# JoshuaLim007/VoxelEngine

Hardware: AMD Instinct MI355X
Metric: Mrays/s primary+1-bounce @1080p, 8k×512×8k brickmap; % HBM roofline (higher is better)
Workload: dtype f32

## Files before the change

voxelengine_amd/csrc/vxrt_persist2.hpp:

```cpp
#pragma once

#include "vxrt_camera.hpp"
#include "vxrt_kernels.hpp"
#include "vxrt_pixel_map.hpp"
#include "vxrt_wave2.hpp"

namespace vxrt {

enum : uint32_t { PX_NONE = 0u, PX_PRIMARY = 1u, PX_SHADOW = 2u, PX_BOUNCE = 3u, PX_BOUNCE2 = 4u };

enum : int { PF_STAGE = 0, PF_TX, PF_ROW, PF_POS_X, PF_POS_Y, PF_POS_Z, PF_COL_X, PF_COL_Y, PF_COL_Z, PF_PCODE, PF_PSTEPS, PF_OCCL,
             PF_SAMPLE, PF_PIXEL_FIELDS };
enum : int { WV_COUNTERS = 0, WV_LIGHT_DX = 4, WV_LIGHT_DY, WV_LIGHT_DZ, WV_LIGHT_IVX, WV_LIGHT_IVY, WV_LIGHT_IVZ, WV_LIGHT_DN,
             WV_LIGHT_STEP_X, WV_LIGHT_STEP_Y, WV_LIGHT_STEP_Z, WV_SHADOW_FROM_END, WV_WORDS = 16 };
#ifndef VXRT_NO_KERNARG_RELOAD
#define VXRT_KERNARG_RELOAD 1
#endif
__device__ __forceinline__ const RenderArgs& kernarg_reload(const RenderArgs& in_registers)
{
#ifdef VXRT_KERNARG_RELOAD
    auto* p = (const __attribute__((address_space(4))) RenderArgs*)__builtin_amdgcn_kernarg_segment_ptr();
    asm volatile("" : "+s"(p));
    return *(const RenderArgs*)p;
#else
    return in_registers;
#endif
}

#ifndef VXRT_PERSIST2_OCC
#define VXRT_PERSIST2_OCC 5
#endif
#ifndef VXRT_QUEUE_GRANULE
#define VXRT_QUEUE_GRANULE 4u
#endif
#ifndef VXRT_SUBROUNDS2
#define VXRT_SUBROUNDS2 3
#endif
#ifndef VXRT_VOTE2_NEXT
#define VXRT_VOTE2_NEXT 2
#endif
#ifndef VXRT_VOTE2_END
#define VXRT_VOTE2_END 1
#endif
#ifndef VXRT_VOTE2_BOX
#define VXRT_VOTE2_BOX 2
#endif
#ifdef VXRT_VOTE2_ABS_BOX
__device__ __forceinline__ bool vote2(int parked, int others, int num, int k)
{
    (void)num;
    return parked >= k || (parked > 0 && others == 0);
}
#else
#define VXRT_VOTE2_ABS_BOX 0
#define VXRT_VOTE2_ABS_END 0
#define VXRT_VOTE2_ABS_NEXT 0
__device__ __forceinline__ bool vote2(int parked, int others, int num, int k)
{
    (void)k;
    return vote_run(parked, others, num);
}
#endif
#define PX_LD_U(f, v) do { if (LDS) v = PX[(f) * 64]; } while (0)
#define PX_ST_U(f, v) do { if (LDS) PX[(f) * 64] = (uint32_t)(v); } while (0)
#define PX_LD_I(f, v) do { if (LDS) v = (int)PX[(f) * 64]; } while (0)
#define PX_LD_F(f, v) do { if (LDS) v = __uint_as_float(PX[(f) * 64]); } while (0)
#define PX_ST_F(f, v) do { if (LDS) PX[(f) * 64] = __float_as_uint(v); } while (0)
#define PX_LD_POS() do { PX_LD_F(PF_POS_X, position.x); PX_LD_F(PF_POS_Y, position.y); PX_LD_F(PF_POS_Z, position.z); } while (0)
#define PX_ST_POS() do { PX_ST_F(PF_POS_X, position.x); PX_ST_F(PF_POS_Y, position.y); PX_ST_F(PF_POS_Z, position.z); } while (0)
#define PX_LD_COL() do { PX_LD_F(PF_COL_X, color.x); PX_LD_F(PF_COL_Y, color.y); PX_LD_F(PF_COL_Z, color.z); } while (0)
#define PX_ST_COL() do { PX_ST_F(PF_COL_X, color.x); PX_ST_F(PF_COL_Y, color.y); PX_ST_F(PF_COL_Z, color.z); } while (0)

template <bool STATS, bool BOUNCE2, bool MULTI, bool WIDE, bool COMMON = false>
__global__ __launch_bounds__(64, VXRT_PERSIST2_OCC) void k_render_persist2(RenderArgs A_kern)
{
    static_assert(!(COMMON && WIDE), "COMMON launches run on ordinary grids");
    using FT = FrameTraits<COMMON>;
    using Tracer = WaveTracerT<WIDE>;
    constexpr bool LDS = true;
    constexpr bool END_SHADOW = !(BOUNCE2 && MULTI) || COMMON;
    __shared__ uint32_t cold_block[(CF_TRACER_FIELDS + PF_PIXEL_FIELDS) * 64 + WV_WORDS];
    const WorldView& W = A_kern.W;
    const int lane = threadIdx.x & 63;
    uint32_t* const PX = &cold_block[CF_TRACER_FIELDS * 64 + lane];
    auto lane_view = [&](const RenderArgs& A, uint32_t v) -> LaneView {
        if (MULTI) {
            const ViewArgs& S = A.views[v];
            return LaneView{S.origin, S.fwd, S.up, S.right, S.frame_number, S.fb, S.color_aov, FT::hit_aov(S.hit_aov)};
        }
        return LaneView{A.origin, A.fwd, A.up, A.right, A.frame_number, A.fb, A.color_aov, FT::hit_aov(A.hit_aov)};
    };

    Tracer T;
    T.init(W, &cold_block[lane]);
    uint32_t stage = PX_NONE;
    uint32_t px_tx = 0, px_row = 0;
    f3 position = mk3(0, 0, 0), color = mk3(0, 0, 0);
    uint32_t pcode = 0;
    int p_steps = 0;
    float occl = 0.0f;
    int sample = 0;
    uint32_t n_primary = 0, n_shadow = 0, n_bounce = 0, n_hits = 0;
    PX_ST_U(PF_STAGE, stage);
    uint32_t* const WV = &cold_block[(CF_TRACER_FIELDS + PF_PIXEL_FIELDS) * 64];
    if (lane < 4)
        WV[WV_COUNTERS + lane] = 0u;
    {
        const f3 lu = A_kern.light_unit;
        const float dd = dot3(lu, lu);
        f3 ld = unit3_ordinary(lu, dd);
        const float ex = ld.x == 0 ? kFltEps : ld.x, ey = ld.y == 0 ? kFltEps : ld.y, ez = ld.z == 0 ? kFltEps : ld.z;
        float lix = rcp_rn(ex), liy = rcp_rn(ey), liz = rcp_rn(ez);
        if (!(ordinary(dd) & ordinary(ex) & ordinary(ey) & ordinary(ez))) {
            ld = unit3(lu);
            lix = 1.0f / (ld.x == 0 ? kFltEps : ld.x);
            liy = 1.0f / (ld.y == 0 ? kFltEps : ld.y);
            liz = 1.0f / (ld.z == 0 ? kFltEps : ld.z);
        }
        const bool light_special = !(fabsf(ld.x) >= kMinFastDir && fabsf(ld.y) >= kMinFastDir && fabsf(ld.z) >= kMinFastDir);
        const bool aov = FT::want_hit_aov(A_kern, MULTI);
        if (lane == 0) {
            WV[WV_LIGHT_DX] = __float_as_uint(ld.x);
            WV[WV_LIGHT_DY] = __float_as_uint(ld.y);
            WV[WV_LIGHT_DZ] = __float_as_uint(ld.z);
            WV[WV_LIGHT_IVX] = __float_as_uint(lix);
            WV[WV_LIGHT_IVY] = __float_as_uint(liy);
            WV[WV_LIGHT_IVZ] = __float_as_uint(liz);
            WV[WV_LIGHT_DN] = (ld.x > 0 ? 0u : 1u) | (ld.y > 0 ? 0u : 2u) | (ld.z > 0 ? 0u : 4u);
            WV[WV_LIGHT_STEP_X] = __float_as_uint(A_kern.light_step.x);
            WV[WV_LIGHT_STEP_Y] = __float_as_uint(A_kern.light_step.y);
            WV[WV_LIGHT_STEP_Z] = __float_as_uint(A_kern.light_step.z);
            WV[WV_SHADOW_FROM_END] = (END_SHADOW && FT::mode(A_kern) == 0 && A_kern.shadow && !light_special && !aov) ? 1u : 0u;
        }
    }

    uint32_t tile = 0, tile_used = 64u, tile_view = 0;
    uint32_t queue_shard = blockIdx.x % kQueueShards;
    bool drained = false;
    unsigned long long dg_iters = 0, dg_walk = 0, dg_drain = 0;
    unsigned int dg_runs[3] = {0, 0, 0}, dg_lanes[3] = {0, 0, 0};
    const unsigned long long dg_t0 = STATS ? wall_clock64() : 0ull;
    unsigned long long dg_next_ticks = 0, dg_park_ticks = 0;
    unsigned long long dg_co_runs = 0, dg_co_starts = 0;
    unsigned long long dg_end_shadow = 0;
#ifdef VXRT_TAIL_DEBUG
    unsigned long long px_t0 = 0;
#endif


    auto store_pixel = [&](const RenderArgs& A, const PixelCoords& pc, const LaneView& V, f3 origin, bool hit, f3 normal, f3 pos, f3 shaded) {
        PixelSink sink{A, pc.out_row, V.fb, V.color_aov};
        const int Wd = (int)A.width, Hd = (int)A.height;
        if (hit) {
            if (FT::mode(A) == 1) {
                f3 dv = pos - origin;
                float dist = sqrtf(dot3(dv, dv));
                const float wrap = (float)(1.0 + 1e-6);
                f3 hp = mk3(fmodf(pos.x / 128.0f, wrap), fmodf(pos.y / 128.0f, wrap), fmodf(pos.z / 128.0f, wrap));
                if (pc.x < (Wd >> 1) && pc.y < (Hd >> 1))
                    sink.put(pc.x, pc.y, normal);
                else if (pc.x >= (Wd >> 1) && pc.y < (Hd >> 1))
                    sink.put(pc.x, pc.y, hp);
                else if (pc.x < (Wd >> 1)) {
// ... 10 lines not shown
                    c = mk3(shaded.x / (shaded.x + 1.0f), shaded.y / (shaded.y + 1.0f), shaded.z / (shaded.z + 1.0f));
                c = mk3(lo(hi(c.x, 0), 1), lo(hi(c.y, 0), 1), lo(hi(c.z, 0), 1));
                sink.put(pc.x, pc.y, c);
            }
        } else {
            sink.put(pc.x, pc.y, shaded);
        }
        if (pc.tx == (A.width >> 1) && pc.ty == (A.height >> 1)) {
            float ten = 10.0f;
            pin(ten);
            sink.put(pc.x, pc.y, mk3(ten, ten, ten));
        }
        if (FT::mode(A) == 1 && pc.x < (Wd >> 1) && pc.y > (Hd >> 1))
            sink.put(pc.x, pc.y, mk3((float)p_steps / 256.0f, 0, 0));
    };

    auto shadow_from_end = [&](Tracer& Tr, const lanemask_t ended) -> lanemask_t {
        if (ended == 0ull)
            return 0ull;
        bool go = false;
        if (lane_test(ended)) {
            if (PX[PF_STAGE * 64] == PX_PRIMARY && WV[WV_SHADOW_FROM_END] != 0u) {
                TraceResult r;
                Tr.result(W, r);
                const f3 at = r.pos;
                const f3 from = at + mk3(__uint_as_float(WV[WV_LIGHT_STEP_X]), __uint_as_float(WV[WV_LIGHT_STEP_Y]),
                                         __uint_as_float(WV[WV_LIGHT_STEP_Z]));
                const f3 s0 = mk3(from.x * W.inv_f, from.y * W.inv_f, from.z * W.inv_f);
                const uint32_t signs = __float_as_uint(s0.x) | __float_as_uint(s0.y) | __float_as_uint(s0.z);
                if ((int32_t)signs >= 0 && s0.x < (float)W.cx && s0.y < (float)W.cy && s0.z < (float)W.cz) {
                    PX[PF_PCODE * 64] = r.ncode;
                    PX[PF_PSTEPS * 64] = (uint32_t)r.steps;
                    PX[PF_POS_X * 64] = __float_as_uint(at.x);
                    PX[PF_POS_Y * 64] = __float_as_uint(at.y);
                    PX[PF_POS_Z * 64] = __float_as_uint(at.z);
                    PX[PF_COL_X * 64] = 0u;
                    PX[PF_COL_Y * 64] = 0u;
                    PX[PF_COL_Z * 64] = 0u;
                    PX[PF_STAGE * 64] = PX_SHADOW;
                    Tr.cold[CF_RAY_CODES * 64] = (uint32_t)kMaxSteps << 7;
                    Tr.cold[CF_START_X * 64] = __float_as_uint(s0.x);
                    Tr.cold[CF_START_Y * 64] = __float_as_uint(s0.y);
                    Tr.cold[CF_START_Z * 64] = __float_as_uint(s0.z);
                    Tr.cold[CF_LAST_CI * 64] = 0xFFFFFFFFu;
                    Tr.cold[CF_TOTAL * 64] = 0u;
                    Tr.d = mk3(__uint_as_float(WV[WV_LIGHT_DX]), __uint_as_float(WV[WV_LIGHT_DY]), __uint_as_float(WV[WV_LIGHT_DZ]));
                    Tr.ivx = __uint_as_float(WV[WV_LIGHT_IVX]);
                    Tr.ivy = __uint_as_float(WV[WV_LIGHT_IVY]);
                    Tr.ivz = __uint_as_float(WV[WV_LIGHT_IVZ]);
                    Tr.dn = WV[WV_LIGHT_DN];
                    Tr.special = false;
                    Tr.st = ST_WALK;
                    go = true;
                }
            }
        }
        const lanemask_t launched = __ballot(go);
        const uint32_t n = (uint32_t)__popcll(launched);
        if (lane == 0) {
            WV[WV_COUNTERS + 1] += n;
            WV[WV_COUNTERS + 3] += n;
        }
        if (STATS)
            dg_end_shadow += n;
        return launched;
    };

    for (;;) {
        const unsigned long long m_walk = __ballot(T.st == ST_WALK);
        const unsigned long long m_box = __ballot(T.st == ST_BOX);
        const unsigned long long m_end = __ballot(waits_for_end(T.st));
        const unsigned long long m_next = __ballot(T.st == ST_DONE);
        if ((m_walk | m_box | m_end | m_next) == 0ull)
            break;
        const int n_walk = __popcll(m_walk), n_box = __popcll(m_box), n_end = __popcll(m_end), n_next = __popcll(m_next);
        if (STATS) {
            dg_iters += 1;
            dg_walk += (unsigned long long)n_walk;
            dg_drain += drained ? 1ull : 0ull;
        }

        int c_walk = n_walk, c_box = n_box, c_end = n_end, c_next = n_next;
        bool dg_end_ran = false, dg_end_restarted = false;
        if (vote2(c_box, c_walk, VXRT_VOTE2_BOX, VXRT_VOTE2_ABS_BOX)) {
            if (STATS) {
                dg_runs[2] += 1u;
                dg_lanes[2] += (unsigned)c_box;
                dg_park_ticks -= wall_clock64();
            }
            T.template phase_box<STATS>(W);
            if (STATS)
                dg_park_ticks += wall_clock64();
            c_box = 0;
            c_walk = __popcll(__ballot(T.st == ST_WALK));
            c_end = __popcll(__ballot(waits_for_end(T.st)));
        }
        if (vote2(c_end, c_walk + c_box, VXRT_VOTE2_END, VXRT_VOTE2_ABS_END)) {
            if (STATS) {
                dg_runs[1] += 1u;
                dg_lanes[1] += (unsigned)c_end;
                dg_park_ticks -= wall_clock64();
            }
            if constexpr (END_SHADOW)
                T.template phase_end_deferred<STATS>(W, shadow_from_end);
            else
                T.template phase_end_deferred<STATS>(W);
            if (STATS)
                dg_park_ticks += wall_clock64();
            c_end = 0;
            c_walk = __popcll(__ballot(T.st == ST_WALK));
            if (STATS) {
                dg_end_ran = true;
                dg_end_restarted = T.pend_m != 0ull;
            }
            c_next = __popcll(__ballot(T.st == ST_DONE));
        }
        if (vote2(c_next, c_walk + c_box + c_end, VXRT_VOTE2_NEXT, VXRT_VOTE2_ABS_NEXT)) {
            if (STATS) {
                dg_runs[0] += 1u;
                dg_lanes[0] += (unsigned)c_next;
                dg_next_ticks -= wall_clock64();
            }
            const RenderArgs& A = kernarg_reload(A_kern);
            const uint32_t ntx = (A.width + 7u) / 8u, nty = (A.launch_rows + 7u) / 8u, ntiles = ntx * nty;
            const f3 L = A.light_dir;
            const f3 sray = A.light_unit;
            PX_LD_U(PF_STAGE, stage);
            PX_LD_U(PF_TX, px_tx);
            PX_LD_U(PF_ROW, px_row);
            bool launch = false;
            bool c_hit = false, c_shadow = false, c_bounce = false;
            f3 l_origin = mk3(0, 0, 0), l_dir = mk3(1, 0, 0);
            int l_max = kMaxSteps;
            if (T.st == ST_DONE && stage != PX_NONE) {
                const LaneView V = lane_view(A, MULTI ? px_row >> 16 : 0u);
                const PixelCoords pc = pixel_coords<COMMON>(A, V.frame_number, px_tx, MULTI ? px_row & 0xFFFFu : px_row);
                const f3 origin = camera_origin<FT>(A, V, pc.x, pc.y);
                TraceResult r;
                T.result(W, r);
                bool finalize = false, do_shade = false, shadowed = false, bounce = false, bounce2 = false;
                if (stage == PX_PRIMARY) {
                    pcode = r.ncode;
                    p_steps = r.steps;
                    position = r.pos;
                    PX_ST_U(PF_PCODE, pcode);
                    PX_ST_U(PF_PSTEPS, p_steps);
                    PX_ST_POS();
                    if (V.hit_aov)
                        V.hit_aov[(size_t)pc.out_row * A.width + (size_t)pc.x] =
                            r.hit ? (long long)r.vx + (long long)W.X * ((long long)r.vy + (long long)W.Y * (long long)r.vz) : -1ll;
                    c_hit = r.hit;
                    if (r.hit) {
                        color = mk3(0, 0, 0);
                        PX_ST_COL();
                    }
                    if (!(r.hit && FT::mode(A) == 0)) {
                        stage = r.hit ? PX_PRIMARY : PX_NONE;
                        finalize = true;
                    } else if (A.shadow) {
                        c_shadow = true;
                        launch = true;
                        l_origin = position + A.light_step;
                        l_dir = sray;
                        l_max = kMaxSteps;
                        stage = PX_SHADOW;
                    } else {
                        do_shade = true;
// ... 99 lines not shown
                    }
#endif
                    stage = PX_NONE;
                }
            }
            bool got = false;
            uint32_t new_tx = 0, new_row = 0;
            unsigned long long want = __ballot(T.st == ST_DONE && stage == PX_NONE);
            while (want != 0ull && !drained) {
                if (tile_used >= 64u) {
                    tile = queue_take(A.tile_counter, ntiles * (MULTI ? A.nviews : 1u), VXRT_QUEUE_GRANULE, queue_shard, lane);
                    if (tile == kQueueDry) {
                        drained = true;
                        break;
                    }
                    tile_used = 0u;
                    if (MULTI) {
                        tile_view = tile / ntiles;
                        tile -= tile_view * ntiles;
                        const ViewArgs& S = A.views[tile_view];
                        if (S.row_order_n)
                            tile = (uint32_t)S.row_order[tile / ntx] * ntx + tile % ntx;
                    } else if (A.tile_order) {
                        tile = A.tile_order[tile];
                    } else if (A.row_order_n) {
                        tile = (uint32_t)A.row_order[tile / ntx] * ntx + tile % ntx;
                    }
                }
                const uint32_t avail = 64u - tile_used;
                const bool wants = ((want >> lane) & 1ull) != 0ull;
                const uint32_t rank = __builtin_amdgcn_mbcnt_hi((uint32_t)(want >> 32), __builtin_amdgcn_mbcnt_lo((uint32_t)want, 0u));
                if (wants && rank < avail) {
                    const uint32_t p = tile_used + rank;
                    new_tx = (tile % ntx) * 8u + (p & 7u);
                    new_row = (tile / ntx) * 8u + (p >> 3);
                    got = pixel_coords<COMMON>(A, MULTI ? A.views[tile_view].frame_number : A.frame_number, new_tx, new_row).live;
                    if (MULTI)
                        new_row |= tile_view << 16;
                }
                const uint32_t asked = (uint32_t)__popcll(want);
                tile_used += asked < avail ? asked : avail;
                want = __ballot(T.st == ST_DONE && stage == PX_NONE && !got);
            }
            if (got) {
                PX_ST_U(PF_TX, new_tx);
                PX_ST_U(PF_ROW, new_row);
                const LaneView V = lane_view(A, MULTI ? new_row >> 16 : 0u);
                const PixelCoords pc = pixel_coords<COMMON>(A, V.frame_number, new_tx, MULTI ? new_row & 0xFFFFu : new_row);
                camera_ray<FT>(A, V, pc.x, pc.y, l_origin, l_dir);
                color = l_dir;
                PX_ST_COL();
                l_max = kMaxSteps;
                launch = true;
                stage = PX_PRIMARY;
#ifdef VXRT_TAIL_DEBUG
                px_t0 = wall_clock64();
#endif
            }
            if (launch)
                T.begin_ray_deferred(W, l_origin, l_dir, l_max);
            T.after_begin_ray_deferred(launch);
            if (STATS) {
                dg_co_runs += dg_end_ran ? 1ull : 0ull;
                dg_co_starts += (dg_end_restarted && __ballot(launch) != 0ull) ? 1ull : 0ull;
            }
            if (drained && T.st == ST_DONE && stage == PX_NONE)
                T.st = ST_IDLE;
            PX_ST_U(PF_STAGE, stage);
            {
                const uint32_t d0 = (uint32_t)__popcll(__ballot(got)), d1 = (uint32_t)__popcll(__ballot(c_shadow)),
                               d2 = (uint32_t)__popcll(__ballot(c_bounce)), d3 = (uint32_t)__popcll(__ballot(c_hit));
                if (lane == 0) {
                    uint32_t* const C = &WV[WV_COUNTERS];
                    C[0] += d0;
                    C[1] += d1;
                    C[2] += d2;
                    C[3] += d3;
                }
            }
            if (STATS)
                dg_next_ticks += wall_clock64();
        }

        T.start_pending(W);
        T.template probe_pairs<VXRT_SUBROUNDS2, STATS>(W);
    }

    if (lane == 0) {
        const uint32_t* const C = &WV[WV_COUNTERS];
        n_primary = C[0];
        n_shadow = C[1];
        n_bounce = C[2];
        n_hits = C[3];
    }
    const unsigned long long s0 = n_primary, s1 = n_shadow, s2 = n_bounce, s3 = n_hits;
    unsigned long long* const stats = A_kern.stats ? stats_row_of<kStatRows, kStatRowStride>(A_kern.stats, blockIdx.x) : nullptr;
    if (lane == 0 && stats) {
        atomicAdd(&stats[kStatPrimary], s0);
        atomicAdd(&stats[kStatShadow], s1);
        atomicAdd(&stats[kStatBounce], s2);
        atomicAdd(&stats[kStatPrimaryHits], s3);
    }
    if (STATS) {
        const unsigned long long p0 = wave_sum(T.cnt.coarse_probes), p1 = wave_sum(T.cnt.brick_entries), p2 = wave_sum(T.cnt.fine_probes);
        const unsigned long long g0 = wave_sum(T.cnt.slack_loads), g1 = wave_sum(T.cnt.stray_loads);
        if (lane == 0 && stats) {
            atomicAdd(&stats[kStatCoarseProbes], p0);
            atomicAdd(&stats[kStatBrickEntries], p1);
            atomicAdd(&stats[kStatFineProbes], p2);
            atomicAdd(&stats[kStatGuardSlack], g0);
            atomicAdd(&stats[kStatGuardStray], g1);
            atomicAdd(&stats[kStatDbgIters], dg_iters);
            atomicAdd(&stats[kStatDbgWalkLanes], dg_walk);
            atomicAdd(&stats[kStatDbgNextRuns], (unsigned long long)dg_runs[0]);
            atomicAdd(&stats[kStatDbgEndRuns], (unsigned long long)dg_runs[1]);
            atomicAdd(&stats[kStatDbgBoxRuns], (unsigned long long)dg_runs[2]);
            atomicAdd(&stats[kStatDbgNextLanes], (unsigned long long)dg_lanes[0]);
            atomicAdd(&stats[kStatDbgEndLanes], (unsigned long long)dg_lanes[1]);
            atomicAdd(&stats[kStatDbgBoxLanes], (unsigned long long)dg_lanes[2]);
            atomicAdd(&stats[kStatDbgLifetime], wall_clock64() - dg_t0);
            atomicAdd(&stats[kStatDbgDrained], dg_drain);
            atomicAdd(&stats[kStatDbgNextTicks], dg_next_ticks);
            atomicAdd(&stats[kStatDbgParkTicks], dg_park_ticks);
            atomicAdd(&stats[kStatDbgCoRuns], dg_co_runs);
            atomicAdd(&stats[kStatDbgCoStarts], dg_co_starts);
            atomicAdd(&stats[kStatDbgEndShadow], dg_end_shadow);
        }
    }
}
#undef PX_LD_U
#undef PX_ST_U
#undef PX_LD_I
#undef PX_LD_F
#undef PX_ST_F
#undef PX_LD_POS
#undef PX_ST_POS
#undef PX_LD_COL
#undef PX_ST_COL

}
```

voxelengine_amd/csrc/vxrt_wave2.hpp:

```cpp
#pragma once

#include "vxrt_device.hpp"
#include <type_traits>
#ifdef VXRT_HOST_DEBUG
#include <cstdio>
#include <cstdlib>
#endif

namespace vxrt {

enum : uint32_t { ST_WALK = 0u, ST_BOX = 1u, ST_END = 2u, ST_ENDHIT = 3u, ST_DONE = 4u, ST_IDLE = 5u };
__device__ __forceinline__ bool waits_for_end(uint32_t st) { return (st | 1u) == 3u; }
#ifndef VXRT_PROBE_GD
#define VXRT_PROBE_GD 0
#endif
#ifdef VXRT_HOST_CHECK
inline unsigned long long& host_unsuspected_exits() { static unsigned long long n = 0; return n; }
#endif

__device__ __forceinline__ f3 normal_decode(uint32_t c)
{
    float v = (c & 4u) ? -1.0f : 1.0f;
    uint32_t a = c & 3u;
    return mk3(a == 1u ? v : 0.0f, a == 2u ? v : 0.0f, a == 3u ? v : 0.0f);
// ... 167 lines not shown
    }

    template <bool FINE>
    __device__ __forceinline__ void start_walk(const WorldView& W, const f3 s)
    {
        ws = s;
        const int dmx = FINE ? W.f : W.cx, dmy = FINE ? W.f : W.cy, dmz = FINE ? W.f : W.cz;
        const uint32_t row = (uint32_t)(FINE ? W.f_row : W.c_row), slice = (uint32_t)(FINE ? W.f_slice : W.c_slice);
        const uint32_t nx = 0u - (dn & 1u), ny = 0u - ((dn >> 1) & 1u), nz = 0u - (dn >> 2);
        const uint32_t mx = ~nx, my = ~ny, mz = ~nz;
        const int c_x = f2i(s.x), c_y = f2i(s.y), c_z = f2i(s.z);
        const float xx = (float)(c_x + (int)(nx + 1u)) - s.x, xy = (float)(c_y + (int)(ny + 1u)) - s.y,
                    xz = (float)(c_z + (int)(nz + 1u)) - s.z;
        tn_x = fast_div(xx, d.x, ivx);
        tn_y = fast_div(xy, d.y, ivy);
        tn_z = fast_div(xz, d.z, ivz);
        bool zero_on_face = false;
        if (__ballot(special) != 0ull) {
            if (special) {
                tn_x = d.x != 0 ? xx / d.x : kInf;
                tn_y = d.y != 0 ? xy / d.y : kInf;
                tn_z = d.z != 0 ? xz / d.z : kInf;
                zero_on_face = (d.x == 0 && c_x == dmx) || (d.y == 0 && c_y == dmy) || (d.z == 0 && c_z == dmz);
            }
        }
        const uint32_t fx = ((uint32_t)c_x ^ mx) + (mx & (uint32_t)dmx), fy = ((uint32_t)c_y ^ my) + (my & (uint32_t)dmy),
                       fz = ((uint32_t)c_z ^ mz) + (mz & (uint32_t)dmz);
        const bool inside = fx < (uint32_t)dmx - nx && fy < (uint32_t)dmy - ny && fz < (uint32_t)dmz - nz && !zero_on_face;
        uint32_t px = fx, py = fy, pz = fz;
        if (!FINE && WIDE) {
            constexpr uint32_t cap = ((uint32_t)kMaxSteps - 1u) / 3u;
            px = min(fx, min(cap, kFieldCapXZ));
            py = min(fy, min(cap, kFieldCapY));
            pz = min(fz, min(cap, kFieldCapXZ));
            cold[CF_OFF_XZ * 64] = (fx - px) | ((fz - pz) << 16);
            cold[CF_OFF_Y * 64] = fy - py;
        }
        rem = rp = rpp = inside ? (px | (py << 11) | (pz << 21)) : 0u;
        rem0 = inside ? px + py + pz : 0u;
        const int q_x = clamp_cell(c_x, dmx - 1), q_y = clamp_cell(c_y, dmy - 1), q_z = clamp_cell(c_z, dmz - 1);
        idx = cell_index(q_x, q_y, q_z, (int)row, dmz) + slice;
        di_x = nx | 1u;
        di_z = (row ^ nz) - nz;
        di_y = (slice ^ ny) - ny;
        const uint32_t ex = (uint32_t)(c_x - q_x), ey = (uint32_t)(c_y - q_y), ez = (uint32_t)(c_z - q_z);
        bool single = special;
        fix = 0u;
        if (__ballot(inside && (ex | ey | ez) != 0u) != 0ull) {
            const bool a0 = tn_x < tn_y && tn_x < tn_z;
            const bool a1 = !(tn_x < tn_y) && tn_y < tn_z;
            const bool a2 = !a0 && !a1;
            const uint32_t npend = ex + ey + ez;
            const bool simple = npend == 1u && ((ex != 0u && a0) || (ey != 0u && a1) || (ez != 0u && a2));
            fix = simple ? (((0u - ex) & di_x) | ((0u - ey) & di_y) | ((0u - ez) & di_z)) : 0u;
            single = single || (npend != 0u && !simple);
        }
        const uint32_t bxb = __float_as_uint(FINE ? W.ff : W.wmax_x), byb = __float_as_uint(FINE ? W.ff : W.wmax_y),
                       bzb = __float_as_uint(FINE ? W.ff : W.wmax_z);
        const float hx = (__uint_as_float(bxb & mx) - s.x) * ivx, hy = (__uint_as_float(byb & my) - s.y) * ivy,
                    hz = (__uint_as_float(bzb & mz) - s.z) * ivz;
        float hi_t = vmin3(hx, hy, hz);
        hi_t = hi_t - fabsf(hi_t) * (FINE ? kThrEpsFine : kThrEpsCoarse);
        hi_t = special ? -kInf : hi_t;
        if (FINE) {
            const uint32_t out = __float_as_uint(s.x) | __float_as_uint(s.y) | __float_as_uint(s.z) | __float_as_uint(W.ff - s.x) |
                                 __float_as_uint(W.ff - s.y) | __float_as_uint(W.ff - s.z);
            single = single || (int32_t)out < 0;
        }
        t_hi_real = hi_t;
        t_hi = single ? -kInf : hi_t;
        if (!FINE)
            bits = W.coarse_bits - (slice >> 5);
        st = inside ? (uint32_t)ST_WALK : (uint32_t)ST_END;
    }

    __device__ __forceinline__ void start_pending(const WorldView& W)
    {
        if (pend_m == 0ull)
            return;
        if (lane_pending())
            start_walk<false>(W, mk3(__uint_as_float(cold[CF_START_X * 64]), __uint_as_float(cold[CF_START_Y * 64]),
                                     __uint_as_float(cold[CF_START_Z * 64])));
        pend_m = 0ull;
    }

    __device__ __forceinline__ void begin_ray(const WorldView& W, f3 origin, f3 ray, int max_steps_)
    {
        begin_ray_deferred(W, origin, ray, max_steps_);
        start_walk<false>(W, mk3(__uint_as_float(cold[CF_START_X * 64]), __uint_as_float(cold[CF_START_Y * 64]),
                                 __uint_as_float(cold[CF_START_Z * 64])));
    }
    __device__ __forceinline__ void begin_ray_deferred(const WorldView& W, f3 origin, f3 ray, int max_steps_)
    {
        const float dd = dot3(ray, ray);
        d = unit3_ordinary(ray, dd);
        const float ex = d.x == 0 ? kFltEps : d.x, ey = d.y == 0 ? kFltEps : d.y, ez = d.z == 0 ? kFltEps : d.z;
        ivx = rcp_rn(ex);
        ivy = rcp_rn(ey);
        ivz = rcp_rn(ez);
        if (__ballot(!(ordinary(dd) & ordinary(ex) & ordinary(ey) & ordinary(ez))) != 0ull) {
            d = unit3(ray);
            ivx = 1.0f / (d.x == 0 ? kFltEps : d.x);
            ivy = 1.0f / (d.y == 0 ? kFltEps : d.y);
            ivz = 1.0f / (d.z == 0 ? kFltEps : d.z);
        }
        f3 s0 = mk3(origin.x * W.inv_f, origin.y * W.inv_f, origin.z * W.inv_f);
        uint32_t ec = 0u;
        if (!(s0.x >= 0 && s0.y >= 0 && s0.z >= 0 && s0.x < (float)W.cx && s0.y < (float)W.cy && s0.z < (float)W.cz)) {
            const float e = (float)1e-6;
            f3 p;
            uint32_t c;
            if (slab(s0, mk3(e, e, e), mk3(W.wmax_x, W.wmax_y, W.wmax_z), p, c)) {
                s0 = p;
                ec = c;
            }
        }
        cold[CF_RAY_CODES * 64] = ec | ((uint32_t)max_steps_ << 7);
        cold[CF_START_X * 64] = __float_as_uint(s0.x);
        cold[CF_START_Y * 64] = __float_as_uint(s0.y);
        cold[CF_START_Z * 64] = __float_as_uint(s0.z);
        cold[CF_LAST_CI * 64] = 0xFFFFFFFFu;
        cold[CF_TOTAL * 64] = 0u;
        special = !(fabsf(d.x) >= kMinFastDir && fabsf(d.y) >= kMinFastDir && fabsf(d.z) >= kMinFastDir) ||
                  __float_as_uint(s0.x) == 0x80000000u || __float_as_uint(s0.y) == 0x80000000u || __float_as_uint(s0.z) == 0x80000000u;
        dn = (d.x > 0 ? 0u : 1u) | (d.y > 0 ? 0u : 2u) | (d.z > 0 ? 0u : 4u);
        st = ST_WALK;
    }
    __device__ __forceinline__ void after_begin_ray(bool launched) { fine_m &= ~__ballot(launched); }
    __device__ __forceinline__ void after_begin_ray_deferred(bool launched)
    {
        const lanemask_t m = __ballot(launched);
        fine_m &= ~m;
        pend_m |= m;
    }

    __device__ __forceinline__ f3 cross_of(const WorldView& W, bool fine, uint32_t before, uint32_t dec, float t) const
    {
        int bx, by, bz;
        cells_of(W, fine, before, bx, by, bz);
        const bool on_x = dec == kRemDecX, on_y = dec == kRemDecY, on_z = dec == kRemDecZ;
        float face_x = (float)(bx + (d.x > 0 ? 1 : 0)), face_y = (float)(by + (d.y > 0 ? 1 : 0)), face_z = (float)(bz + (d.z > 0 ? 1 : 0));
        float lin_x = ws.x + (t * d.x), lin_y = ws.y + (t * d.y), lin_z = ws.z + (t * d.z);
        pin(face_x), pin(face_y), pin(face_z), pin(lin_x), pin(lin_y), pin(lin_z);
        return mk3(on_x ? face_x : lin_x, on_y ? face_y : lin_y, on_z ? face_z : lin_z);
    }

    __device__ __forceinline__ void walk_on(const WorldView& W, bool is_fine, bool lin_inside)
    {
        const bool single = t_hi == -kInf;
        if (__ballot(single) == 0ull)
            return;
        int x, y, z;
        cells_of(W, is_fine, rem, x, y, z);
        const int dmx = is_fine ? W.f : W.cx, dmy = is_fine ? W.f : W.cy, dmz = is_fine ? W.f : W.cz;
        const int row = is_fine ? W.f_row : W.c_row, slice = is_fine ? W.f_slice : W.c_slice;
        const uint32_t exact = cell_index(min(x, dmx - 1), min(y, dmy - 1), min(z, dmz - 1), row, dmz) + (uint32_t)slice;
        idx = single ? exact : idx;
        const bool pending = x == dmx || y == dmy || z == dmz;
        t_hi = (single && !pending && lin_inside) ? t_hi_real : t_hi;
    }

    template <bool STATS = false>
    __device__ __forceinline__ void phase_end(const WorldView& W)
    {
        phase_end_deferred<STATS>(W);
        start_pending(W);
// ... 136 lines not shown
                        st = ST_DONE;
                    }
                }
            }
        }
        const lanemask_t m = __ballot(go_coarse);
        fine_m &= ~m;
        pend_m |= m;
        if constexpr (HOOKED) {
            const lanemask_t launched = hook(*this, (lanemask_t)__ballot(ended_hit));
            fine_m &= ~launched;
            pend_m |= launched;
        }
    }

    template <bool STATS = false>
    __device__ __forceinline__ void phase_box(const WorldView& W)
    {
        bool go_fine = false;
        if (st == ST_BOX) {
            int x, y, z;
            cells_of(W, false, rp, x, y, z);
            const int qx = min(x, W.cx - 1), qy = min(y, W.cy - 1), qz = min(z, W.cz - 1);
            const uint32_t ci = cell_index(qx, qy, qz, W.c_row, W.cz);
            const uint2 meta = W.cell_meta[ci];
            const uint32_t e = meta.y;
            const float fqx = (float)qx, fqy = (float)qy, fqz = (float)qz;
            f3 bmin = mk3(((float)(e & 31u) + 0) * W.inv_f + fqx, ((float)((e >> 5) & 31u) + 0) * W.inv_f + fqy,
                          ((float)((e >> 10) & 31u) + 0) * W.inv_f + fqz);
            f3 bmax = mk3(((float)((e >> 15) & 31u) + 1) * W.inv_f + fqx, ((float)((e >> 20) & 31u) + 1) * W.inv_f + fqy,
                          ((float)((e >> 25) & 31u) + 1) * W.inv_f + fqz);
            f3 bp;
            uint32_t bc;
            bool box_hit = slab_fast(ws, bmin, bmax, bp, bc) && bmin.x <= bmax.x;
            if (__ballot(special) != 0ull) {
                if (special)
                    box_hit = slab(ws, bmin, bmax, bp, bc) && bmin.x <= bmax.x;
            }
            if (box_hit) {
                const uint32_t steps = rem0 - rem_sum(rp);
                cold[CF_TOTAL * 64] += steps;
                if (STATS)
                    cnt.coarse_probes += steps + 1u;
                point.x = steps != 0u ? bp.x : ws.x;
                point.y = steps != 0u ? bp.y : ws.y;
                point.z = steps != 0u ? bp.z : ws.z;
                const bool enter = ci != cold[CF_LAST_CI * 64];
                if (enter) {
                    const uint32_t dec = rp - rem;
                    const int axis = dec == kRemDecX ? 0 : (dec == kRemDecY ? 1 : 2);
                    const int packed = axis | ((x - qx) << 2) | ((y - qy) << 3) | ((z - qz) << 4);
                    if (STATS)
                        cnt.brick_entries += 1u;
                    cold[CF_LAST_CI * 64] = ci;
                    cold[CF_CHX * 64] = (uint32_t)qx;
                    cold[CF_CHY * 64] = (uint32_t)qy;
                    cold[CF_CHZ * 64] = (uint32_t)qz;
                    cold[CF_BOX_CODES * 64] = bc | ((uint32_t)packed << 3);
                    const f3 hp = mk3(point.x * W.ff, point.y * W.ff, point.z * W.ff);
                    const f3 ns = mk3(hp.x - fqx * W.ff, hp.y - fqy * W.ff, hp.z - fqz * W.ff);
                    bits = W.pool + (size_t)meta.x * W.brick_words - (W.f_slice >> 5);
                    start_walk<true>(W, ns);
                    go_fine = true;
                } else {
                    st = ST_DONE;
                }
            } else {
                const bool left = (rem & kRemGuards) != 0u;
                if (!left)
                    walk_on(W, false, true);
                st = left ? (uint32_t)ST_END : (uint32_t)ST_WALK;
            }
        }
        fine_m |= __ballot(go_fine);
    }

    template <int PAIRS, bool GUARD = false, bool MASKED = false>
    __device__ __forceinline__ void probe_pairs(const WorldView& W)
    {
#ifdef VXRT_HOST_CHECK
        for (int p = 0; p < 2 * PAIRS; ++p) {
            if (st != ST_WALK)
                return;
            const uint32_t i1 = idx;
            const uint32_t word = bits[i1 >> 5];
            if (GUARD)
                guard_load(W, bits + (i1 >> 5));
            const bool a0 = tn_x < tn_y && tn_x < tn_z;
            const bool a1 = !(tn_x < tn_y) && tn_y < tn_z;
            tp = tl;
            rpp = rp;
            rp = rem;
            tl = lo(lo(tn_x, tn_y), tn_z);
            if (a0) {
                tn_x += fabsf(ivx);
                idx += di_x;
                rem -= kRemDecX;
            } else if (a1) {
                tn_y += fabsf(ivy);
                idx += di_y;
                rem -= kRemDecY;
            } else {
                tn_z += fabsf(ivz);
                idx += di_z;
                rem -= kRemDecZ;
            }
            if (p == 0) {
                idx -= fix;
                fix = 0u;
            }
            const bool sus = !(tl < t_hi), gd = WIDE && (rem & kRemGuards) != 0u;
            if (!WIDE && (rem & kRemGuards) != 0u && !sus)
                host_unsuspected_exits() += 1;
            const bool solid = ((word >> (i1 & 31u)) & 1u) != 0u;
            if (solid)
                st = lane_fine() ? (uint32_t)ST_ENDHIT : (uint32_t)ST_BOX;
            else if (sus || gd)
                st = ST_END;
        }
#else
        const lanemask_t w0 = lane_mask(st == ST_WALK);
        lanemask_t w = w0, hits = 0ull;
#pragma unroll
        for (int k = 0; k < PAIRS; ++k) {
            lanemask_t sus1, gd1, sus2, gd2;
            const uint32_t i1 = idx;
            const uint32_t* a1 = bits + (i1 >> 5);
            if (MASKED)
                a1 = lane_test(w) ? a1 : W.coarse_bits;
            const uint32_t word1 = *a1;
            if (GUARD)
                guard_load(W, a1);
            advance<WIDE || VXRT_PROBE_GD>(w, sus1, gd1);
            if (k == 0) {
                idx -= fix;
                fix = 0u;
            }
            const uint32_t i2 = idx;
            const uint32_t* a2 = bits + (i2 >> 5);
            if (MASKED)
                a2 = lane_test(w) ? a2 : W.coarse_bits;
            const uint32_t word2 = *a2;
            if (GUARD)
                guard_load(W, a2);
            const lanemask_t h1 = lane_mask(bit_of(word1, i1) != 0u) & w;
            const lanemask_t w2 = w & ~(h1 | sus1 | gd1);
            advance<WIDE || VXRT_PROBE_GD>(w2, sus2, gd2);
            const lanemask_t h2 = lane_mask(bit_of(word2, i2) != 0u) & w2;
            hits |= h1 | h2;
            w = w2 & ~(h2 | sus2 | gd2);
        }
        const lanemask_t other = (w0 & ~w) & ~hits;
        const lanemask_t park = hits & ~fine_m, lhit = hits & fine_m;
        asm volatile("s_mov_b64 exec, %[park]\n\t"
                     "v_mov_b32 %[st], 1\n\t"
                     "s_mov_b64 exec, %[lhit]\n\t"
                     "v_mov_b32 %[st], 3\n\t"
                     "s_mov_b64 exec, %[other]\n\t"
                     "v_mov_b32 %[st], 2\n\t"
                     "s_mov_b64 exec, -1"
                     : [st] "+v"(st)
                     : [park] "s"(park), [lhit] "s"(lhit), [other] "s"(other));
        static_assert(ST_BOX == 1u && ST_ENDHIT == 3u && ST_END == 2u, "state codes of the asm above");
#endif
    }

    __device__ __forceinline__ void guard_load(const WorldView& W, const uint32_t* a)
    {
        const uint32_t in_table = (uint32_t)(a >= W.coarse_bits) & (uint32_t)(a < W.coarse_end) | (uint32_t)(a >= W.pool) & (uint32_t)(a < W.pool_end);
        const uint32_t addressable = (uint32_t)(a >= W.coarse_lo) & (uint32_t)(a < W.coarse_hi) | (uint32_t)(a >= W.pool_lo) & (uint32_t)(a < W.pool_hi);
        cnt.slack_loads += (in_table ^ 1u) & addressable;
        cnt.stray_loads += addressable ^ 1u;
    }

#ifndef VXRT_HOST_CHECK
#define VXRT_ADVANCE_ASM(GUARD_PART)                                                                                     \
            "s_mov_b64 exec, %[w]\n\t"                                                                                   \
                                                    \
            "v_cmp_lt_f32 s[84:85], %[tx], %[ty]\n\t"                                                                    \
            "v_cmp_lt_f32 s[86:87], %[tx], %[tz]\n\t"                                                                    \
            "v_cmp_lt_f32 s[88:89], %[ty], %[tz]\n\t"                                                                    \
               \
               \
            "v_mov_b32 %[tp], %[tl]\n\t"                                                                                 \
            "v_mov_b32 %[rpp], %[rp]\n\t"                                                                                \
            "v_mov_b32 %[rp], %[rem]\n\t"                                                                                \
            "v_min3_f32 %[tl], %[tx], %[ty], %[tz]\n\t"                                                                  \
            "v_cmp_nlt_f32 %[sus], %[tl], %[thi]\n\t"                                                                    \
                                                           \
            "s_and_b64 exec, s[84:85], s[86:87]\n\t"                                                                     \
            "v_add_f32 %[tx], %[tx], |%[ivx]|\n\t"                                                                       \
            "v_add_u32 %[idx], %[idx], %[dix]\n\t"                                                                       \
            "v_add_u32 %[rem], -1, %[rem]\n\t"                                                                           \
                                                                             \
            "s_andn2_b64 s[86:87], %[w], exec\n\t"                                                                       \
            "s_andn2_b64 exec, s[88:89], s[84:85]\n\t"                                                                   \
            "v_add_f32 %[ty], %[ty], |%[ivy]|\n\t"                                                                       \
            "v_add_u32 %[idx], %[idx], %[diy]\n\t"                                                                       \
            "v_add_u32 %[rem], 0xfffff800, %[rem]\n\t"                                                                   \
                                                                                      \
            "s_andn2_b64 exec, s[86:87], exec\n\t"                                                                       \
            "v_add_f32 %[tz], %[tz], |%[ivz]|\n\t"                                                                       \
            "v_add_u32 %[idx], %[idx], %[diz]\n\t"                                                                       \
            "v_add_u32 %[rem], 0xffe00000, %[rem]\n\t"                                                                   \
            GUARD_PART                                                                                                    \
            "s_mov_b64 exec, -1"
    template <bool GD>
    __device__ __forceinline__ void advance(const lanemask_t w, lanemask_t& sus, lanemask_t& gd)
    {
        if (!GD) {
            asm volatile(VXRT_ADVANCE_ASM("")
                         : [tx] "+v"(tn_x), [ty] "+v"(tn_y), [tz] "+v"(tn_z), [idx] "+v"(idx), [rem] "+v"(rem), [rp] "+v"(rp), [rpp] "+v"(rpp),
                           [tl] "+v"(tl), [tp] "+v"(tp), [sus] "=&s"(sus)
                         : [w] "s"(w), [ivx] "v"(ivx), [ivy] "v"(ivy), [ivz] "v"(ivz), [dix] "v"(di_x), [diy] "v"(di_y), [diz] "v"(di_z),
                           [thi] "v"(t_hi)
                         : "s84", "s85", "s86", "s87", "s88", "s89", "scc");
            gd = 0ull;
            return;
        }
        uint32_t tmp;
        asm volatile(VXRT_ADVANCE_ASM("s_mov_b64 exec, %[w]\n\t"
                                      "v_and_b32 %[tmp], 0x80100400, %[rem]\n\t"
                                      "v_cmp_ne_u32 %[gd], 0, %[tmp]\n\t")
                     : [tx] "+v"(tn_x), [ty] "+v"(tn_y), [tz] "+v"(tn_z), [idx] "+v"(idx), [rem] "+v"(rem), [rp] "+v"(rp), [rpp] "+v"(rpp),
                       [tl] "+v"(tl), [tp] "+v"(tp), [sus] "=&s"(sus), [gd] "=&s"(gd), [tmp] "=&v"(tmp)
                     : [w] "s"(w), [ivx] "v"(ivx), [ivy] "v"(ivy), [ivz] "v"(ivz), [dix] "v"(di_x), [diy] "v"(di_y), [diz] "v"(di_z),
                       [thi] "v"(t_hi)
                     : "s84", "s85", "s86", "s87", "s88", "s89", "scc");
    }
#undef VXRT_ADVANCE_ASM
#endif

    __device__ __forceinline__ void result(const WorldView& W, TraceResult& out) const
    {
        const uint32_t ray_codes = cold[CF_RAY_CODES * 64];
        const bool hit = (ray_codes & 0x40u) != 0u;
        const int total_ = (int)cold[CF_TOTAL * 64];
        const int hx = (int)cold[CF_CHX * 64], hy = (int)cold[CF_CHY * 64], hz = (int)cold[CF_CHZ * 64];
        out.hit = hit;
        out.steps = total_;
        const bool is_fine = lane_fine();
        const float ox = (float)hx * W.ff, oy = (float)hy * W.ff, oz = (float)hz * W.ff;
        out.pos = mk3(is_fine ? point.x + ox : point.x * W.ff, is_fine ? point.y + oy : point.y * W.ff,
                      is_fine ? point.z + oz : point.z * W.ff);
        int x, y, z;
        cells_of(W, true, rp, x, y, z);
        out.vx = hx * W.f + min(x, W.f - 1);
        out.vy = hy * W.f + min(y, W.f - 1);
// ... 46 lines not shown
```

Baseline: 9470.

## Run box phase after starting pending rays with a first probe step

For most kernel variants, the box (brick descent) phase moves from the top of the wave scheduling loop to the end. It now runs after pending rays are started, and each newly started ray first does one probe of its initial coarse cell. Rays that hit a solid cell straight away can then join the same box phase instead of waiting a whole loop iteration, which should raise lane occupancy in the divergent phases. The cost is an extra probe step and extra ballots per iteration, and a different phase order that could shift how the vote heuristics behave. The host-check probe path is also factored into a probe_one helper.

```diff
diff --git a/voxelengine_amd/csrc/vxrt_persist2.hpp b/voxelengine_amd/csrc/vxrt_persist2.hpp
--- a/voxelengine_amd/csrc/vxrt_persist2.hpp
+++ b/voxelengine_amd/csrc/vxrt_persist2.hpp
@@ -79,6 +79,7 @@
     using Tracer = WaveTracerT<WIDE>;
     constexpr bool LDS = true;
     constexpr bool END_SHADOW = !(BOUNCE2 && MULTI) || COMMON;
+    constexpr bool BOX_LAST = !(BOUNCE2 && MULTI && !WIDE && !COMMON);
     __shared__ uint32_t cold_block[(CF_TRACER_FIELDS + PF_PIXEL_FIELDS) * 64 + WV_WORDS];
     const WorldView& W = A_kern.W;
     const int lane = threadIdx.x & 63;
@@ -255,7 +256,7 @@
 
         int c_walk = n_walk, c_box = n_box, c_end = n_end, c_next = n_next;
         bool dg_end_ran = false, dg_end_restarted = false;
-        if (vote2(c_box, c_walk, VXRT_VOTE2_BOX, VXRT_VOTE2_ABS_BOX)) {
+        if (!BOX_LAST && vote2(c_box, c_walk, VXRT_VOTE2_BOX, VXRT_VOTE2_ABS_BOX)) {
             if (STATS) {
                 dg_runs[2] += 1u;
                 dg_lanes[2] += (unsigned)c_box;
@@ -521,7 +522,26 @@
                 dg_next_ticks += wall_clock64();
         }
 
-        T.start_pending(W);
+        if constexpr (!BOX_LAST) {
+            T.start_pending(W);
+        } else {
+            const bool set_up = T.pend_m != 0ull;
+            T.template start_pending_probed<STATS>(W);
+            if (set_up) {
+                c_walk = __popcll(__ballot(T.st == ST_WALK));
+                c_box = __popcll(__ballot(T.st == ST_BOX));
+            }
+            if (vote2(c_box, c_walk, VXRT_VOTE2_BOX, VXRT_VOTE2_ABS_BOX)) {
+                if (STATS) {
+                    dg_runs[2] += 1u;
+                    dg_lanes[2] += (unsigned)c_box;
+                    dg_park_ticks -= wall_clock64();
+                }
+                T.template phase_box<STATS>(W);
+                if (STATS)
+                    dg_park_ticks += wall_clock64();
+            }
+        }
         T.template probe_pairs<VXRT_SUBROUNDS2, STATS>(W);
     }
 
diff --git a/voxelengine_amd/csrc/vxrt_wave2.hpp b/voxelengine_amd/csrc/vxrt_wave2.hpp
--- a/voxelengine_amd/csrc/vxrt_wave2.hpp
+++ b/voxelengine_amd/csrc/vxrt_wave2.hpp
@@ -273,6 +273,44 @@
             start_walk<false>(W, mk3(__uint_as_float(cold[CF_START_X * 64]), __uint_as_float(cold[CF_START_Y * 64]),
                                      __uint_as_float(cold[CF_START_Z * 64])));
         pend_m = 0ull;
+    }
+
+    template <bool GUARD = false>
+    __device__ __forceinline__ void start_pending_probed(const WorldView& W)
+    {
+        if (pend_m == 0ull)
+            return;
+        if (lane_pending())
+            start_walk<false>(W, mk3(__uint_as_float(cold[CF_START_X * 64]), __uint_as_float(cold[CF_START_Y * 64]),
+                                     __uint_as_float(cold[CF_START_Z * 64])));
+#ifdef VXRT_HOST_CHECK
+        if (lane_pending())
+            probe_one<GUARD>(W, true);
+        pend_m = 0ull;
+#else
+        const lanemask_t w = pend_m & lane_mask(st == ST_WALK);
+        pend_m = 0ull;
+        const uint32_t i1 = idx;
+        const uint32_t* a1 = bits + (i1 >> 5);
+        const uint32_t word1 = *a1;
+        if (GUARD)
+            guard_load(W, a1);
+        lanemask_t sus, gd;
+        advance<WIDE || VXRT_PROBE_GD>(w, sus, gd);
+        const lanemask_t park = lane_mask(bit_of(word1, i1) != 0u) & w;
+        const lanemask_t other = w & ~park & (sus | gd);
+        asm volatile("s_mov_b64 exec, %[w]\n\t"
+                     "v_sub_u32 %[idx], %[idx], %[fix]\n\t"
+                     "v_mov_b32 %[fix], 0\n\t"
+                     "s_mov_b64 exec, %[park]\n\t"
+                     "v_mov_b32 %[st], 1\n\t"
+                     "s_mov_b64 exec, %[other]\n\t"
+                     "v_mov_b32 %[st], 2\n\t"
+                     "s_mov_b64 exec, -1"
+                     : [st] "+v"(st), [idx] "+v"(idx), [fix] "+v"(fix)
+                     : [w] "s"(w), [park] "s"(park), [other] "s"(other));
+        static_assert(ST_BOX == 1u && ST_END == 2u, "state codes of the asm above");
+#endif
     }
 
     __device__ __forceinline__ void begin_ray(const WorldView& W, f3 origin, f3 ray, int max_steps_)
@@ -575,41 +613,7 @@
         for (int p = 0; p < 2 * PAIRS; ++p) {
             if (st != ST_WALK)
                 return;
-            const uint32_t i1 = idx;
-            const uint32_t word = bits[i1 >> 5];
-            if (GUARD)
-                guard_load(W, bits + (i1 >> 5));
-            const bool a0 = tn_x < tn_y && tn_x < tn_z;
-            const bool a1 = !(tn_x < tn_y) && tn_y < tn_z;
-            tp = tl;
-            rpp = rp;
-            rp = rem;
-            tl = lo(lo(tn_x, tn_y), tn_z);
-            if (a0) {
-                tn_x += fabsf(ivx);
-                idx += di_x;
-                rem -= kRemDecX;
-            } else if (a1) {
-                tn_y += fabsf(ivy);
-                idx += di_y;
-                rem -= kRemDecY;
-            } else {
-                tn_z += fabsf(ivz);
-                idx += di_z;
-                rem -= kRemDecZ;
-            }
-            if (p == 0) {
-                idx -= fix;
-                fix = 0u;
-            }
-            const bool sus = !(tl < t_hi), gd = WIDE && (rem & kRemGuards) != 0u;
-            if (!WIDE && (rem & kRemGuards) != 0u && !sus)
-                host_unsuspected_exits() += 1;
-            const bool solid = ((word >> (i1 & 31u)) & 1u) != 0u;
-            if (solid)
-                st = lane_fine() ? (uint32_t)ST_ENDHIT : (uint32_t)ST_BOX;
-            else if (sus || gd)
-                st = ST_END;
+            probe_one<GUARD>(W, p == 0);
         }
 #else
         const lanemask_t w0 = lane_mask(st == ST_WALK);
@@ -657,6 +661,50 @@
         static_assert(ST_BOX == 1u && ST_ENDHIT == 3u && ST_END == 2u, "state codes of the asm above");
 #endif
     }
+
+#ifdef VXRT_HOST_CHECK
+    template <bool GUARD>
+    __device__ __forceinline__ void probe_one(const WorldView& W, const bool first)
+    {
+        if (st != ST_WALK)
+            return;
+        const uint32_t i1 = idx;
+        const uint32_t word = bits[i1 >> 5];
+        if (GUARD)
+            guard_load(W, bits + (i1 >> 5));
+        const bool a0 = tn_x < tn_y && tn_x < tn_z;
+        const bool a1 = !(tn_x < tn_y) && tn_y < tn_z;
+        tp = tl;
+        rpp = rp;
+        rp = rem;
+        tl = lo(lo(tn_x, tn_y), tn_z);
+        if (a0) {
+            tn_x += fabsf(ivx);
+            idx += di_x;
+            rem -= kRemDecX;
+        } else if (a1) {
+            tn_y += fabsf(ivy);
+            idx += di_y;
+            rem -= kRemDecY;
+        } else {
+            tn_z += fabsf(ivz);
+            idx += di_z;
+            rem -= kRemDecZ;
+        }
+        if (first) {
+            idx -= fix;
+            fix = 0u;
+        }
+        const bool sus = !(tl < t_hi), gd = WIDE && (rem & kRemGuards) != 0u;
+        if (!WIDE && (rem & kRemGuards) != 0u && !sus)
+            host_unsuspected_exits() += 1;
+        const bool solid = ((word >> (i1 & 31u)) & 1u) != 0u;
+        if (solid)
+            st = lane_fine() ? (uint32_t)ST_ENDHIT : (uint32_t)ST_BOX;
+        else if (sus || gd)
+            st = ST_END;
+    }
+#endif
 
     __device__ __forceinline__ void guard_load(const WorldView& W, const uint32_t* a)
     {
```

New measurement: 9621 (median of 6 runs). 1.02x the previous value.
